# avik-pal/RegNeuralDE.jl

Hardware: AMD Instinct MI355X
Metric: training-step samples/sec + mean NFE, MNIST Neural ODE bs=512 (higher is better)
Workload: dtype f32; 1 GPU; MNIST NODE regularized (error_est), Tsit5 reltol=abstol=1.4e-8, batch 512 per GPU, 1xMI355X per rank; step = loss fwd + reverse pass through the solver + InvDecay/Momentum update; the weights train during the timed steps (mean_nfe drifts with --steps: value_fixed_weights of --full is the stationary companion); global_batch=512, parallelism=single

## Files before the change

regneuralde.jl_amd/csrc/rnde_reverse.hip:

```cpp
#include "rnde_node.h"
#include "rnde_wgradx.h"

static rnde_status chain_bwd_run(rnde_node* h, const float* u_bar_dev, const float* saveval_bar_host, float* x_bar_dev,
                                 float* p_bar_dev, float* tspan_bar_host, hipStream_t s, bool sync = true, float* tspan_bar_dev = nullptr);
static rnde_status bwd_run(rnde_node* h, const float* u_bar_dev, const float* saveval_bar_host, float* x_bar_dev,
                           float* p_bar_dev, float* tspan_bar_host, hipStream_t s, bool sync = true, float* tspan_bar_dev = nullptr);


extern "C" rnde_status rnde_node_backward_async(rnde_node* h, const float* u_bar_dev, const float* saveval_bar_host, float* x_bar_dev,
                                                float* p_bar_dev, float* tspan_bar_dev, void* stream) {
    if (!h) return RNDE_ERR_BAD_ARG;
    if (!h->have_tape) { h->err = "no recorded forward"; return RNDE_ERR_NO_TAPE; }
    if (h->engine == 3) return chain_bwd_run(h, u_bar_dev, saveval_bar_host, x_bar_dev, p_bar_dev, nullptr, (hipStream_t)stream, false, tspan_bar_dev);
    return bwd_run(h, u_bar_dev, saveval_bar_host, x_bar_dev, p_bar_dev, nullptr, (hipStream_t)stream, false, tspan_bar_dev);
}

extern "C" rnde_status rnde_node_backward(rnde_node* h, const float* u_bar_dev, const float* saveval_bar_host,
                                          float* x_bar_dev, float* p_bar_dev, float* tspan_bar_host, void* stream) {
    if (!h) return RNDE_ERR_BAD_ARG;
    if (!h->have_tape) { h->err = "no recorded forward"; return RNDE_ERR_NO_TAPE; }
    if (h->engine == 3) return chain_bwd_run(h, u_bar_dev, saveval_bar_host, x_bar_dev, p_bar_dev, tspan_bar_host, (hipStream_t)stream);
    return bwd_run(h, u_bar_dev, saveval_bar_host, x_bar_dev, p_bar_dev, tspan_bar_host, (hipStream_t)stream);
}
extern "C" rnde_status rnde_node_backward_host(rnde_node* h, const float* u_bar, const float* saveval_bar, float* x_bar,
                                               float* p_bar, float* tspan_bar) {
    if (!h) return RNDE_ERR_BAD_ARG;
    float *ub = nullptr, *xb = nullptr, *pb = nullptr;
    const size_t nb = (size_t)h->D * h->B * 4;
    HIPCHK(h, hipMalloc((void**)&ub, nb)); HIPCHK(h, hipMalloc((void**)&xb, nb)); HIPCHK(h, hipMalloc((void**)&pb, (size_t)h->P * 4));
    HIPCHK(h, hipMemcpy(ub, u_bar, nb, hipMemcpyHostToDevice));
    rnde_status st = rnde_node_backward(h, ub, saveval_bar, xb, pb, tspan_bar, nullptr);
    if (st == RNDE_OK) { hipMemcpy(x_bar, xb, nb, hipMemcpyDeviceToHost); hipMemcpy(p_bar, pb, (size_t)h->P * 4, hipMemcpyDeviceToHost); }
    hipFree(ub); hipFree(xb); hipFree(pb);
    return st;
}

static rnde_status bwd_prepare(rnde_node* h) {
    BwdBuffers& b = h->bw;
    if (b.ready) return RNDE_OK;
    const size_t A = (size_t)h->D * h->Bpad_max, HB = (size_t)h->H * h->Bpad_max;
    const int cap = h->cfg.max_attempts;
    HIPCHK(h, hipMalloc((void**)&b.U, A * 4)); HIPCHK(h, hipMalloc((void**)&b.K1, A * 4)); HIPCHK(h, hipMalloc((void**)&b.UB1, A * 4));
    HIPCHK(h, hipMalloc((void**)&b.zi2, 2 * A * 4)); HIPCHK(h, hipMalloc((void**)&b.zi1, 2 * HB * 4));
    HIPCHK(h, hipMalloc((void**)&b.svb_att, (size_t)cap * 4));
    HIPCHK(h, hipMalloc((void**)&b.bstate, 2 * sizeof(BState) + 64)); HIPCHK(h, hipMalloc((void**)&b.ibstate, 2 * sizeof(IBState)));
    HIPCHK(h, hipMalloc((void**)&b.bpart, (size_t)(2 * h->nwg_max + 256) * 4 * 4)); HIPCHK(h, hipMalloc((void**)&b.ipart, (size_t)2 * h->nwg_max * 4 * 4));
    HIPCHK(h, hipMalloc((void**)&b.tspan_out, 2 * 4));
    const size_t nev = (size_t)6 * cap + 2;
    const size_t desc_blob = 2 * nev * sizeof(EvalDesc) + (size_t)cap * 4 + 64;
    HIPCHK(h, hipMalloc((void**)&b.ev1, desc_blob)); HIPCHK(h, hipMalloc((void**)&b.ev2, nev * sizeof(EvalDesc)));
    HIPCHK(h, hipHostMalloc((void**)&b.h_ev1, desc_blob)); HIPCHK(h, hipHostMalloc((void**)&b.h_ev2, nev * sizeof(EvalDesc)));
    HIPCHK(h, hipHostMalloc((void**)&b.h_svb, (size_t)cap * 4));
    const size_t seg = std::max((size_t)h->H * (h->D + 2), (size_t)h->D * (h->H + 2));
    b.slab_floats = seg * 256;
    HIPCHK(h, hipMalloc((void**)&b.slab, 2 * b.slab_floats * 4));
    HIPCHK(h, hipMalloc((void**)&b.slab_r, 2 * 16 * seg * 4));
    if (!h->wstream) {
        int prio_least = 0, prio_greatest = 0;
        (void)hipDeviceGetStreamPriorityRange(&prio_least, &prio_greatest);
        HIPCHK(h, hipStreamCreateWithPriority(&h->wstream, hipStreamNonBlocking, prio_least));
        h->wevents.resize(66);
        for (auto& e : h->wevents) HIPCHK(h, hipEventCreateWithFlags(&e, hipEventDisableTiming));
    }
    if (h->engine == 2) {
        HIPCHK(h, hipMalloc((void**)&b.UTB, A * 4)); HIPCHK(h, hipMalloc((void**)&b.UNB, A * 4)); HIPCHK(h, hipMalloc((void**)&b.UPB0, A * 4));
        HIPCHK(h, hipMalloc((void**)&b.GB, 15 * A * 4));
    }
    b.ready = true;
    return RNDE_OK;
}

static bool wgrad3_ok(int M, int Nx) {
    const bool tall = M >= Nx;
    const int wide = tall ? M : Nx + 2, narrow = tall ? Nx + 2 : M;
    return getenv("RNDE_WGRAD_LEGACY") == nullptr && getenv("RNDE_WGRAD_V2") == nullptr && M % 4 == 0 && Nx % 4 == 0 && wide > 656 &&
           wide <= 800 && narrow <= 112;
}
static rnde_status launch_wgrad_part(rnde_node* h, const EvalDesc* ev, int n_evals, int per_chunk, int M, int Nx, int Bpad,
                                     float* slab, int* chunk_cursor, hipStream_t s, int max_chunks = 0) {
    if (n_evals <= 0) return RNDE_OK;
    const int mtiles = (M + 31) / 32, ntiles = (Nx + 2 + 31) / 32;
    const bool tall = M >= Nx;
    const int MB = tall ? 2 : 4, NB = tall ? 4 : 2;
    const int blocks = ((mtiles + MB - 1) / MB) * ((ntiles + NB - 1) / NB);
    const long long len = (long long)M * (Nx + 2);
    const int chunks = (n_evals + per_chunk - 1) / per_chunk;
    float* dst = slab + (size_t)(*chunk_cursor) * len;
    static const bool legacy = getenv("RNDE_WGRAD_LEGACY") != nullptr;
    const bool fits = tall ? (Nx + 2 <= 128) : (M <= 128);
    if (wgrad3_ok(M, Nx)) {
        const int total_steps = n_evals * ((Bpad + 31) / 32);
        static const int target_chunks = getenv("RNDE_WGRAD3_CHUNKS") ? atoi(getenv("RNDE_WGRAD3_CHUNKS")) : 128;
        int sc = std::max(1, std::min({max_chunks > 0 ? max_chunks : target_chunks, total_steps, 256}));
        const int steps_per_chunk = (total_steps + sc - 1) / sc;
        sc = (total_steps + steps_per_chunk - 1) / steps_per_chunk;
        if ((size_t)(*chunk_cursor + sc) * (size_t)len > h->bw.slab_floats) { h->err = "weight-gradient slab overflow"; return RNDE_ERR_BAD_ARG; }
        const bool x3_off = getenv("RNDE_X3_WGRAD_OFF") != nullptr;
        const bool x3_half = getenv("RNDE_X3_WGRAD_HALF") != nullptr;
        const int TT4 = ((tall ? M : Nx + 2) + 15) / 16;
        if (h->x3_packed && !x3_off && !x3_half && TT4 >= 28 && TT4 <= 52) {
            static const int target4 = getenv("RNDE_WGRAD4_CHUNKS") ? atoi(getenv("RNDE_WGRAD4_CHUNKS")) : 64;
            int sc4 = std::max(1, std::min({max_chunks > 0 ? max_chunks / 2 : target4, total_steps, 256}));
            const int spc4 = (total_steps + sc4 - 1) / sc4;
            sc4 = (total_steps + spc4 - 1) / spc4;
            if ((size_t)(*chunk_cursor + sc4) * (size_t)len > h->bw.slab_floats) { h->err = "weight-gradient slab overflow"; return RNDE_ERR_BAD_ARG; }
            static DeviceOnce attr4;
            if (attr4.need()) {
                HIPCHK(h, hipFuncSetAttribute((const void*)rnde_wgrad4x_kernel<true>, hipFuncAttributeMaxDynamicSharedMemorySize, (int)kWx4LdsBytes));
                HIPCHK(h, hipFuncSetAttribute((const void*)rnde_wgrad4x_kernel<false>, hipFuncAttributeMaxDynamicSharedMemorySize, (int)kWx4LdsBytes));
                attr4.done();
            }
            const dim3 g4(32 * ((sc4 + 7) / 8));
            if (tall) hipLaunchKernelGGL((rnde_wgrad4x_kernel<true>), g4, dim3(448), kWx4LdsBytes, s, ev, n_evals, spc4, sc4, M, Nx, Bpad, dst);
            else hipLaunchKernelGGL((rnde_wgrad4x_kernel<false>), g4, dim3(448), kWx4LdsBytes, s, ev, n_evals, spc4, sc4, M, Nx, Bpad, dst);
            HIPCHK(h, hipGetLastError());
            *chunk_cursor += sc4;
            return RNDE_OK;
        }
        if (h->x3_packed && !x3_off) {
            static DeviceOnce attrx;
            if (attrx.need()) {
                HIPCHK(h, hipFuncSetAttribute((const void*)rnde_wgrad3x_kernel<true>, hipFuncAttributeMaxDynamicSharedMemorySize, (int)kWxLdsBytes));
                HIPCHK(h, hipFuncSetAttribute((const void*)rnde_wgrad3x_kernel<false>, hipFuncAttributeMaxDynamicSharedMemorySize, (int)kWxLdsBytes));
                attrx.done();
            }
            if (tall) hipLaunchKernelGGL((rnde_wgrad3x_kernel<true>), dim3(2, sc), dim3(448), kWxLdsBytes, s, ev, n_evals, steps_per_chunk, M, Nx, Bpad, dst);
            else hipLaunchKernelGGL((rnde_wgrad3x_kernel<false>), dim3(2, sc), dim3(448), kWxLdsBytes, s, ev, n_evals, steps_per_chunk, M, Nx, Bpad, dst);
            HIPCHK(h, hipGetLastError());
            *chunk_cursor += sc;
            return RNDE_OK;
        }
        const size_t lds = (size_t)2 * 32 * (464 + 144) * sizeof(float);
        static DeviceOnce attr;
        if (attr.need()) {
            HIPCHK(h, hipFuncSetAttribute((const void*)rnde_wgrad3_kernel<true>, hipFuncAttributeMaxDynamicSharedMemorySize, (int)lds));
            HIPCHK(h, hipFuncSetAttribute((const void*)rnde_wgrad3_kernel<false>, hipFuncAttributeMaxDynamicSharedMemorySize, (int)lds));
            attr.done();
        }
        if (tall) hipLaunchKernelGGL((rnde_wgrad3_kernel<true>), dim3(2, sc), dim3(448), lds, s, ev, n_evals, steps_per_chunk, M, Nx, Bpad, dst);
        else hipLaunchKernelGGL((rnde_wgrad3_kernel<false>), dim3(2, sc), dim3(448), lds, s, ev, n_evals, steps_per_chunk, M, Nx, Bpad, dst);
        HIPCHK(h, hipGetLastError());
        *chunk_cursor += sc;
        return RNDE_OK;
    }
    if (!legacy && fits) {
        const int pblocks = tall ? (M + 127) / 128 : (Nx + 2 + 127) / 128;
        const int total_steps = n_evals * ((Bpad + 31) / 32);
        static const int target_wgs = getenv("RNDE_WGRAD_WGS") ? atoi(getenv("RNDE_WGRAD_WGS")) : 768;
        int sc = std::max(1, std::min({target_wgs / pblocks, total_steps, 256}));
        const int steps_per_chunk = (total_steps + sc - 1) / sc;
        sc = (total_steps + steps_per_chunk - 1) / steps_per_chunk;
        if ((size_t)(*chunk_cursor + sc) * (size_t)len > h->bw.slab_floats) { h->err = "weight-gradient slab overflow"; return RNDE_ERR_BAD_ARG; }
        if (tall) hipLaunchKernelGGL((rnde_wgrad2_kernel<true>), dim3(pblocks, sc), dim3(256), 0, s, ev, n_evals, steps_per_chunk, M, Nx, Bpad, dst);
        else hipLaunchKernelGGL((rnde_wgrad2_kernel<false>), dim3(pblocks, sc), dim3(256), 0, s, ev, n_evals, steps_per_chunk, M, Nx, Bpad, dst);
        HIPCHK(h, hipGetLastError());
        *chunk_cursor += sc;
        return RNDE_OK;
    } else {
        if ((size_t)(*chunk_cursor + chunks) * (size_t)len > h->bw.slab_floats) { h->err = "weight-gradient slab overflow"; return RNDE_ERR_BAD_ARG; }
        if (tall) hipLaunchKernelGGL((rnde_wgrad_kernel<2, 4>), dim3(blocks, chunks), dim3(64), 0, s, ev, n_evals, per_chunk, M, Nx, Bpad, dst);
        else hipLaunchKernelGGL((rnde_wgrad_kernel<4, 2>), dim3(blocks, chunks), dim3(64), 0, s, ev, n_evals, per_chunk, M, Nx, Bpad, dst);
    }
    HIPCHK(h, hipGetLastError());
    *chunk_cursor += chunks;
    return RNDE_OK;
}
static rnde_status launch_wgrad_reduce(rnde_node* h, const float* slab, int chunks, int M, int Nx, float* out, hipStream_t s) {
    const long long len = (long long)M * (Nx + 2);
    const int grid = (int)std::min<long long>((len + 255) / 256, 2048);
    if (chunks <= 16) {
        hipLaunchKernelGGL(rnde_wgrad_reduce, dim3(grid, 1), dim3(256), 0, s, slab, chunks, chunks, len, out);
    } else {
        const int per_group = (chunks + 15) / 16, groups = (chunks + per_group - 1) / per_group;
        hipLaunchKernelGGL(rnde_wgrad_reduce, dim3(grid, groups), dim3(256), 0, s, slab, chunks, per_group, len, h->bw.slab_r);
        hipLaunchKernelGGL(rnde_wgrad_reduce, dim3(grid, 1), dim3(256), 0, s, (const float*)h->bw.slab_r, groups, groups, len, out);
    }
    HIPCHK(h, hipGetLastError());
    return RNDE_OK;
}

static rnde_status bwd_run(rnde_node* h, const float* u_bar_dev, const float* saveval_bar_host, float* x_bar_dev,
                           float* p_bar_dev, float* tspan_bar_host, hipStream_t s, bool sync, float* tspan_bar_dev) {
    HIPCHK(h, hipSetDevice(h->cfg.device));
    rnde_status st = bwd_prepare(h);
    if (st != RNDE_OK) return st;
    BwdBuffers& b = h->bw;
    int n_att = h->n_att;
    const float svb_scale = h->couple ? (float)h->couple_world : 1.f;
    for (int i = 0; i < n_att; ++i)
        b.h_svb[i] = (saveval_bar_host && h->sv_index[i] >= 0) ? svb_scale * saveval_bar_host[h->sv_index[i]] : 0.f;
    const int ne_all = 2 + 6 * n_att;
    EvalDesc* const h_ev1 = b.h_ev1; EvalDesc* const h_ev2 = b.h_ev1 + ne_all; float* const h_svb_blob = (float*)(b.h_ev1 + 2 * (size_t)ne_all);
    EvalDesc* const d_ev1 = b.ev1;   EvalDesc* const d_ev2 = b.ev1 + ne_all;   float* const d_svb = (float*)(b.ev1 + 2 * (size_t)ne_all);
    memcpy(h_svb_blob, b.h_svb, (size_t)n_att * 4);
    BwdParams Q{};
    Q.F = make_params(h, h->xcopy, h->B, h->t0, h->t1, 1);
    Q.U = b.U; Q.K1 = b.K1; Q.UB1 = b.UB1; Q.zi2 = b.zi2; Q.zi1 = b.zi1; Q.svb_att = d_svb;
    Q.bstate = b.bstate; Q.ibstate = b.ibstate; Q.bpart = b.bpart; Q.ipart = b.ipart;
    Q.ubar = u_bar_dev; Q.xbar = x_bar_dev; Q.tspan_out = b.tspan_out;
    Q.n_att = n_att; Q.track_ctrl = h->cfg.track_ctrl; Q.track_initdt = h->cfg.track_initdt; Q.reg_kind = h->cfg.regularize;
    Q.bpart_n = Q.F.nwg;
    Q.tspan_scale = h->couple ? 1.f / (float)h->couple_world : 1.f;
#ifdef RNDE_DIAG
    if (getenv("RNDE_DIAG_BWD")) { if (!h->diag_buf) hipMalloc((void**)&h->diag_buf, 8192); hipMemset(h->diag_buf, 0, 512); Q.F.dbg_out = h->diag_buf; }
#endif
    Q.sv_T = (int)h->saveat.size();
    Q.sv_ubar0 = (!h->saveat.empty() && h->saveat[0] == h->t0) ? u_bar_dev : nullptr;
    if (!h->saveat.empty() && h->engine != 2) { h->err = "saveat reverse pass runs on the stage engine only"; return RNDE_ERR_BAD_ARG; }
    const long long A = (long long)h->D * Q.F.Bpad, HB = (long long)h->H * Q.F.Bpad;
    RecLayout L{A, HB};
    int ne = 2;
    h_ev2[0] = EvalDesc{b.zi2, h->h0, h->t0, 0};           h_ev1[0] = EvalDesc{b.zi1, h->xcopy, h->t0, 0};
    h_ev2[1] = EvalDesc{b.zi2 + A, h->h1, h->t0 + h->h_init->dt0, 0}; h_ev1[1] = EvalDesc{b.zi1 + HB, h->u1, h->t0 + h->h_init->dt0, 0};
    for (int n = 0; n < n_att; ++n) {
        const StepMeta& m = h->h_meta[n];
        const float* R = h->arena + (long long)m.rec * h->rec_stride;
        for (int sidx = 2; sidx <= 7; ++sidx) {
            const float ts = m.t + tsC(sidx - 1) * m.dt;
            h_ev2[ne] = EvalDesc{R + L.k(sidx), R + L.h(sidx), ts, 0};
            h_ev1[ne] = EvalDesc{R + L.z1(sidx), sidx < 7 ? R + L.g(sidx) : R + L.unew(), ts, 0};
            ++ne;
        }
    }
    HIPCHK(h, hipMemcpyAsync(b.ev1, b.h_ev1, 2 * (size_t)ne * sizeof(EvalDesc) + (size_t)n_att * 4, hipMemcpyHostToDevice, s));
    float* slab1 = b.slab;
    float* slab2w = b.slab + b.slab_floats;
    int cur1 = 0, cur2 = 0, evi = 0;
    const int per_chunk = std::max(1, (ne + 239) / 240);
    const int side_pct = h->wgrad_side_pct;
    const int sweep_cus = 8 * h->sR * ((Q.F.Bpad / 16 + 7) / 8);
    const bool side = h->engine == 2 && h->persist == 1 && side_pct > 0 && n_att >= 8 && sweep_cus <= 224 &&
                      wgrad3_ok(h->H, h->D) && wgrad3_ok(h->D, h->H);
    const int side_att = side ? std::min(n_att, n_att * side_pct / 100) : 0;
    const int group = std::max(4, (side_att + 5) / 6);
    bool used_side = false;
    auto wgrad_group = [&](int lo, int hi, bool on_side) -> rnde_status {
        if (hi <= lo) return RNDE_OK;
        hipStream_t ws = s;
        if (on_side) {
            hipEvent_t ev = h->wevents[evi++ % 64];
            HIPCHK(h, hipEventRecord(ev, s));
            HIPCHK(h, hipStreamWaitEvent(h->wstream, ev, 0));
            ws = h->wstream; used_side = true;
        }
        rnde_status r = launch_wgrad_part(h, d_ev1 + lo, hi - lo, per_chunk, h->H, h->D, h->B, slab1, &cur1, ws, on_side ? 16 : 0);
        if (r != RNDE_OK) return r;
        return launch_wgrad_part(h, d_ev2 + lo, hi - lo, per_chunk, h->D, h->H, h->B, slab2w, &cur2, ws, on_side ? 16 : 0);
    };
    int hi_att = n_att;
    hipError_t e;
    h->tev_bwd = false;
    if (h->timing) HIPCHK(h, hipEventRecord(h->tev[2], s));
    if (h->engine == 2) {
        if (!h->rev_packed) {
            HIPCHK(h, stage_pack(h, h->pcopy, h->spwBt, 2, h->sMT, h->sKHb, s));
            HIPCHK(h, stage_pack(h, h->pcopy, h->spwDt, 3, h->sHT, h->sMT, s));
        }
        h->rev_packed = false;
        BStageParams BQ{};
        BQ.B = Q; BQ.p = h->pcopy; BQ.pwBt = h->spwBt; BQ.pwDt = h->spwDt; BQ.slab = h->slab2; BQ.x3Bt = h->x3Bt; BQ.x3Dt = h->x3Dt;
        BQ.UTB = b.UTB; BQ.UNB = b.UNB; BQ.UPB0 = b.UPB0; BQ.GB = b.GB;
        BQ.EXK = b.GB + 6 * A; BQ.EXG = b.GB + 7 * A; BQ.SVW = b.GB + 8 * A;
        BQ.sv_t = h->saveat.empty() ? nullptr : h->sv_t_dev; BQ.sv_ubar = u_bar_dev; BQ.nsave = (int)h->saveat.size();
        BQ.MT = h->sMT; BQ.WT = h->sWT; BQ.R = h->sR; BQ.C = Q.F.Bpad / 16; BQ.HT = h->sHT; BQ.KHb = h->sKHb;
        double* const bsum = (double*)(b.bstate + 2);
        const bool pre_reduce = h->persist == 1 && Q.bpart_n >= 896 && !getenv("RNDE_NO_BPART_REDUCE");
        if (pre_reduce) BQ.B.bsum = bsum;
        const dim3 grid(BQ.R * BQ.C), blk(64 * BQ.WT);
        std::vector<int> sv_lo(n_att, 0), sv_hi(n_att, 0);
        if (!h->saveat.empty()) {
            int ns = (h->saveat[0] == h->t0) ? 1 : 0;
            for (int n = 0; n < n_att; ++n) {
                sv_lo[n] = ns;
                if (h->h_meta[n].flags & F_ACCEPT) {
                    const float tnew = h->h_meta[n].t + h->h_meta[n].dt;
                    while (ns < (int)h->saveat.size() && h->saveat[ns] <= tnew) ++ns;
                }
                sv_hi[n] = ns;
            }
        }
        auto eig_coefs = [&](int n, float& c1, float& c2) {
            c1 = 0.f; c2 = 0.f;
            const StepMeta& mm = h->h_meta[n];
            const bool eg_ok = !(mm.eigen == 0.f || mm.eigen != mm.eigen);
            double eigb = 0.0;
            if (h->cfg.regularize == RNDE_REG_STIFF && eg_ok) eigb = (double)b.h_svb[n] * (mm.eigen > 0 ? 1.0 : -1.0) / 3.5068;
            if (h->cfg.regularize == RNDE_REG_ERR_STIFF && eg_ok) eigb = 0.1 * (double)b.h_svb[n] / 3.5068;
            if (h->cfg.regularize == RNDE_REG_STIFF_DT && eg_ok) eigb = (double)b.h_svb[n] * ((double)mm.eigen * (double)mm.dt > 0 ? 1.0 : -1.0) * (double)mm.dt;
            if (eigb != 0.0 && mm.n1 > 0.f && mm.n2 > 0.f) {
                c1 = (float)(eigb / ((double)mm.n2 * (double)mm.n1));
                c2 = (float)(-eigb * ((double)mm.n1 / (double)mm.n2) / ((double)mm.n2 * (double)mm.n2));
            }
        };
        for (int n = n_att - 1; n >= 0; --n) {
            float c1 = 0.f, c2 = 0.f;
            eig_coefs(n, c1, c2);
            const double qo = pow((double)h->h_meta[n].qold_in, (double)kBeta2);
            if (h->persist == 1) {
                PersistSync Y{h->tslab, h->pabort, h->pxcc, h->persist_spins};
                HIPCHK(h, slab_prepare(h, Q.F.Bpad, s));
                const dim3 pgrid(8 * BQ.R * ((BQ.C + 7) / 8));
                const bool fix = BQ.WT == 7 && BQ.HT == 7 && BQ.KHb == 7 && BQ.MT == 49 && BQ.R == 7 && h->D == 784 && h->H == 100 && !h->stage_generic;
                if (fix) {
                    const size_t flds = h->stage_lds + (size_t)(RNDE_BSTAGE_HDMA ? 1 : 0) * 6 * 7 * 2 * 1024;
                    static DeviceOnce attr;
                    if (attr.need()) {
                        HIPCHK(h, hipFuncSetAttribute((const void*)rnde_bstage_attempt_kernel<1, 1>, hipFuncAttributeMaxDynamicSharedMemorySize, 160 * 1024));
                        HIPCHK(h, hipFuncSetAttribute((const void*)rnde_bstage_attempt_kernel<0, 1>, hipFuncAttributeMaxDynamicSharedMemorySize, 160 * 1024));
                        attr.done();
                    }
                    const bool x3 = h->x3_packed && h->x3Bt && h->x3Dt && !getenv("RNDE_X3_REV_OFF");
                    if (x3) {
                        const size_t xlds = sizeof(float) * ((size_t)2 * kX3ImageFloats + 64) + (size_t)(RNDE_BSTAGE_HDMA ? 1 : 0) * 6 * 7 * 2 * 1024;
                        static DeviceOnce attr3;
                        if (attr3.need()) {
#define RNDE_X3_ATTR(A, E) HIPCHK(h, hipFuncSetAttribute((const void*)rnde_bstage_attempt_kernel<A, 1, 1, E>, hipFuncAttributeMaxDynamicSharedMemorySize, 160 * 1024));
                            RNDE_X3_ATTR(1, 0) RNDE_X3_ATTR(1, 1) RNDE_X3_ATTR(1, 2) RNDE_X3_ATTR(1, 3) RNDE_X3_ATTR(0, 0) RNDE_X3_ATTR(0, 1) RNDE_X3_ATTR(0, 2) RNDE_X3_ATTR(0, 3)
#undef RNDE_X3_ATTR
                            attr3.done();
                        }
                        const int ex = (h->saveat.empty() ? 0 : 1) | (h->cfg.regularize >= RNDE_REG_STIFF ? 2 : 0);
#define RNDE_X3_LAUNCH(A, E) hipLaunchKernelGGL((rnde_bstage_attempt_kernel<A, 1, 1, E>), pgrid, blk, xlds, s, BQ, n, h->h_meta[n], c1, c2, sv_lo[n], sv_hi[n], Y, qo, b.h_svb[n])
                        if (h->act2) { if (ex == 0) RNDE_X3_LAUNCH(1, 0); else if (ex == 1) RNDE_X3_LAUNCH(1, 1); else if (ex == 2) RNDE_X3_LAUNCH(1, 2); else RNDE_X3_LAUNCH(1, 3); }
                        else { if (ex == 0) RNDE_X3_LAUNCH(0, 0); else if (ex == 1) RNDE_X3_LAUNCH(0, 1); else if (ex == 2) RNDE_X3_LAUNCH(0, 2); else RNDE_X3_LAUNCH(0, 3); }
#undef RNDE_X3_LAUNCH
                    } else if (h->act2) hipLaunchKernelGGL((rnde_bstage_attempt_kernel<1, 1>), pgrid, blk, flds, s, BQ, n, h->h_meta[n], c1, c2, sv_lo[n], sv_hi[n], Y, qo, b.h_svb[n]);
                    else hipLaunchKernelGGL((rnde_bstage_attempt_kernel<0, 1>), pgrid, blk, flds, s, BQ, n, h->h_meta[n], c1, c2, sv_lo[n], sv_hi[n], Y, qo, b.h_svb[n]);
                } else if (h->act2) hipLaunchKernelGGL((rnde_bstage_attempt_kernel<1, 0>), pgrid, blk, h->stage_lds, s, BQ, n, h->h_meta[n], c1, c2, sv_lo[n], sv_hi[n], Y, qo, b.h_svb[n]);
                else hipLaunchKernelGGL((rnde_bstage_attempt_kernel<0, 0>), pgrid, blk, h->stage_lds, s, BQ, n, h->h_meta[n], c1, c2, sv_lo[n], sv_hi[n], Y, qo, b.h_svb[n]);
                if ((st = couple_sum(h, b.bpart + (size_t)(n & 1) * Q.bpart_n * 4, 4LL * Q.bpart_n, s)) != RNDE_OK) return st;
                if (pre_reduce && n > 0) hipLaunchKernelGGL(rnde_bpart_reduce_kernel, dim3(1), dim3(64), 0, s, Q, n, bsum);
                if (n >= n_att - side_att && (hi_att - n >= group || n == n_att - side_att)) {
                    st = wgrad_group(2 + 6 * n, 2 + 6 * hi_att, true);
                    if (st != RNDE_OK) return st;
                    hi_att = n;
                }
                continue;
            }
            if (h->act2) hipLaunchKernelGGL((rnde_bstage_kernel<1, BM_START>), grid, blk, h->stage_lds, s, BQ, n, 0, h->h_meta[n], c1, c2, sv_lo[n], sv_hi[n], qo);
            else hipLaunchKernelGGL((rnde_bstage_kernel<0, BM_START>), grid, blk, h->stage_lds, s, BQ, n, 0, h->h_meta[n], c1, c2, sv_lo[n], sv_hi[n], qo);
            for (int j = 6; j >= 1; --j) {
                if (h->act2) hipLaunchKernelGGL((rnde_bstage_kernel<1, BM_STAGE>), grid, blk, h->stage_lds, s, BQ, n, j, h->h_meta[n], c1, c2, sv_lo[n], sv_hi[n], qo);
                else hipLaunchKernelGGL((rnde_bstage_kernel<0, BM_STAGE>), grid, blk, h->stage_lds, s, BQ, n, j, h->h_meta[n], c1, c2, sv_lo[n], sv_hi[n], qo);
            }
            if ((st = couple_sum(h, b.bpart + (size_t)(n & 1) * Q.bpart_n * 4, 4LL * Q.bpart_n, s)) != RNDE_OK) return st;
        }
        HIPCHK(h, hipGetLastError());
        {
            if (h->act2) {
                hipLaunchKernelGGL((rnde_binit_stage_kernel<1, 0>), grid, blk, h->stage_lds, s, BQ);
                hipLaunchKernelGGL((rnde_binit_stage_kernel<1, 1>), grid, blk, h->stage_lds, s, BQ);
            } else {
                hipLaunchKernelGGL((rnde_binit_stage_kernel<0, 0>), grid, blk, h->stage_lds, s, BQ);
                hipLaunchKernelGGL((rnde_binit_stage_kernel<0, 1>), grid, blk, h->stage_lds, s, BQ);
            }
            if ((st = couple_sum(h, Q.ipart, 4LL * Q.F.nwg, s)) != RNDE_OK) return st;
            if (h->act2) {
                hipLaunchKernelGGL((rnde_binit_stage_kernel<1, 2>), grid, blk, h->stage_lds, s, BQ);
                hipLaunchKernelGGL((rnde_binit_stage_kernel<1, 3>), grid, blk, h->stage_lds, s, BQ);
            } else {
                hipLaunchKernelGGL((rnde_binit_stage_kernel<0, 2>), grid, blk, h->stage_lds, s, BQ);
                hipLaunchKernelGGL((rnde_binit_stage_kernel<0, 3>), grid, blk, h->stage_lds, s, BQ);
            }
            if ((st = couple_sum(h, Q.ipart + 4LL * Q.F.nwg, 4LL * Q.F.nwg, s)) != RNDE_OK) return st;
            hipLaunchKernelGGL(rnde_bfin_kernel, dim3(1), dim3(64), 0, s, Q);
            HIPCHK(h, hipGetLastError());
        }
    }
    if (h->timing) HIPCHK(h, hipEventRecord(h->tev[3], s));
    st = wgrad_group(0, 2 + 6 * hi_att, false);
    if (st != RNDE_OK) return st;
    if (used_side) {
        hipEvent_t ev = h->wevents[64];
        HIPCHK(h, hipEventRecord(ev, h->wstream));
        HIPCHK(h, hipStreamWaitEvent(s, ev, 0));
    }
    if (cur1 > 16 && cur2 > 16) {
        const long long len1 = (long long)h->H * (h->D + 2), len2 = (long long)h->D * (h->H + 2);
        const size_t seg_r = std::max((size_t)len1, (size_t)len2);
        float* r1 = b.slab_r; float* r2 = b.slab_r + 16 * seg_r;
        const int pg1 = (cur1 + 15) / 16, g1 = (cur1 + pg1 - 1) / pg1, pg2 = (cur2 + 15) / 16, g2 = (cur2 + pg2 - 1) / pg2;
        const int grid = (int)std::min<long long>((std::max(len1, len2) + 255) / 256, 2048);
        ReducePair A{{{slab1, r1, len1, cur1, pg1}, {slab2w, r2, len2, cur2, pg2}}};
        hipLaunchKernelGGL(rnde_wgrad_reduce_pair, dim3(grid, std::max(g1, g2), 2), dim3(256), 0, s, A);
        ReducePair Bp{{{r1, p_bar_dev, len1, g1, g1}, {r2, p_bar_dev + (size_t)h->H * (h->D + 2), len2, g2, g2}}};
        hipLaunchKernelGGL(rnde_wgrad_reduce_pair, dim3(grid, 1, 2), dim3(256), 0, s, Bp);
        HIPCHK(h, hipGetLastError());
    } else {
        st = launch_wgrad_reduce(h, slab1, cur1, h->H, h->D, p_bar_dev, s);
        if (st != RNDE_OK) return st;
        st = launch_wgrad_reduce(h, slab2w, cur2, h->D, h->H, p_bar_dev + (size_t)h->H * (h->D + 2), s);
        if (st != RNDE_OK) return st;
    }
    if (h->timing) { HIPCHK(h, hipEventRecord(h->tev[4], s)); h->tev_bwd = true; }
#ifdef RNDE_DIAG
    if (h->engine == 2 && h->persist == 1 && getenv("RNDE_DIAG_BWD")) {
        unsigned long long hst[64] = {0};
        hipStreamSynchronize(s);
        hipMemcpy(hst, h->diag_buf, sizeof(hst), hipMemcpyDeviceToHost);
        fprintf(stderr, "persistent reverse attempt (workgroup 0 thread 0, cycles): START %lld (entry->weights issued %lld, ->w1t %lld, ->array loads issued %lld, finish_attempt_scalars %lld, scalar chain %lld, vector part %lld), its phase D + put %lld\n", (long long)(hst[1]-hst[0]), (long long)(hst[43]-hst[0]), (long long)(hst[44]-hst[43]), (long long)(hst[40]-hst[44]), (long long)(hst[41]-hst[40]), (long long)(hst[42]-hst[41]), (long long)(hst[1]-hst[42]), (long long)(hst[2]-hst[1]));
        for (int st = 0; st < 6; ++st) { const unsigned long long* q = hst + 3 + 5 * st; const unsigned long long prev = st == 0 ? hst[2] : hst[7 + 5 * (st - 1)];
            fprintf(stderr, "  stage j=%d: poll %lld A %lld B %lld C %lld D+put %lld\n", 6 - st, (long long)(q[0]-prev), (long long)(q[1]-q[0]), (long long)(q[2]-q[1]), (long long)(q[3]-q[2]), st < 5 ? (long long)(q[4]-q[3]) : 0LL); }
        fprintf(stderr, "  total %lld cycles to the end of stage 1, END (reduction of the 21 partial sums) %lld; in START's vector part the wait for the record's k arrays %lld\n",
                (long long)(hst[34]-hst[0]), (long long)(hst[35]-hst[34]), (long long)(hst[45]-hst[42]));
    }
#endif
    if (!sync) {
        if (tspan_bar_dev) HIPCHK(h, hipMemcpyAsync(tspan_bar_dev, b.tspan_out, 8, hipMemcpyDeviceToDevice, s));
        h->have_tape = false;
        h->pending_bwd = (h->engine == 2 && h->persist == 1);
        return RNDE_OK;
    }
    HIPCHK(h, hipMemcpyAsync(h->h_scal, b.tspan_out, 8, hipMemcpyDeviceToHost, s));
    if (h->engine == 2) persist_check_enqueue(h, h->sR * (Q.F.Bpad / 16), s);
    HIPCHK(h, hipStreamSynchronize(s));
    if (h->couple && rnde_comm_health(h->couple) != RNDE_OK) { h->err = std::string("coupled controller: ") + rnde_comm_last_error(h->couple); return RNDE_ERR_HIP; }
    if (tspan_bar_host) { tspan_bar_host[0] = h->h_scal[0]; tspan_bar_host[1] = h->h_scal[1]; }
// ... 406 lines not shown
```

regneuralde.jl_amd/csrc/rnde_wgradx.h:

```cpp
#pragma once
#include "rnde_x3.h"

namespace rnde {

constexpr int kWxRowShorts = 40;
constexpr int kWxTallRows = 400, kWxNarrowRows = 112;
constexpr int kWxPlaneShortsT = kWxTallRows * kWxRowShorts, kWxPlaneShortsS = kWxNarrowRows * kWxRowShorts;
constexpr size_t kWxLdsBytes = (size_t)3 * (kWxPlaneShortsT + kWxPlaneShortsS) * 2;

template <bool TALL_IS_Z>
__global__ __launch_bounds__(448) void rnde_wgrad3x_kernel(const EvalDesc* __restrict__ evals, int n_evals, int per_chunk, int M, int Nx, int Bpad, float* __restrict__ slab) {
    constexpr int KC = 32;
    extern __shared__ __attribute__((aligned(16))) unsigned short wxs[];
    unsigned short* TP = wxs;
    unsigned short* SP = wxs + 3 * kWxPlaneShortsT;
    const int tid = threadIdx.x, lane = tid & 63, w = __builtin_amdgcn_readfirstlane(tid >> 6);
    const int mrow = lane & 15, kk = lane >> 4;
    const int TR = TALL_IS_Z ? M : Nx + 2, SR = TALL_IS_Z ? Nx + 2 : M;
    const int TRp = TALL_IS_Z ? M : Nx, SRp = TALL_IS_Z ? Nx : M;
    const int TT = (TR + 15) >> 4, T0 = (TT + 1) >> 1;
    const int half = blockIdx.x, chunk = blockIdx.y;
    const int tile_lo = half ? T0 : 0, tile_hi = half ? TT : T0, ntile = tile_hi - tile_lo;
    const int row_lo = 16 * tile_lo, nrow = 16 * ntile;
    const int steps_per_eval = (Bpad + KC - 1) / KC;
    const int s_lo = chunk * per_chunk, s_hi = min(n_evals * steps_per_eval, s_lo + per_chunk);
    const int total_steps = max(0, s_hi - s_lo);
    x3f4 acc[4][7];
#pragma unroll
    for (int i = 0; i < 4; ++i)
#pragma unroll
        for (int n = 0; n < 7; ++n) acc[i][n] = (x3f4){0.f, 0.f, 0.f, 0.f};
    const bool has3 = w + 21 < ntile;

    constexpr unsigned kNoSrc = 0x7FFFFF00u;
    int u_kind[5], u_dst[5];
    unsigned u_voff[5];
#pragma unroll
    for (int jj = 0; jj < 4; ++jj) {
        const int u = tid + 448 * jj;
        int kind = 0, dst = 0; unsigned voff = kNoSrc;
        if (u < 4 * nrow) {
            const int o = u / nrow, row = u - o * nrow, gr = row_lo + row;
            kind = gr < TRp ? 1 : (!TALL_IS_Z && gr == TRp ? 2 : (!TALL_IS_Z && gr == TRp + 1 ? 3 : 4));
            if (kind == 1) voff = 4u * (unsigned)(gr + 8 * o * TRp);
            dst = row * kWxRowShorts + 8 * o;
        }
        u_kind[jj] = kind; u_voff[jj] = voff; u_dst[jj] = dst;
    }
    {
        const int o = tid / kWxNarrowRows, row = tid - o * kWxNarrowRows;
        const int kind = row < SRp ? 1 : (TALL_IS_Z && row == SRp ? 2 : (TALL_IS_Z && row == SRp + 1 ? 3 : 4));
        u_kind[4] = kind; u_voff[4] = kind == 1 ? 4u * (unsigned)(row + 8 * o * SRp) : kNoSrc;
        u_dst[4] = 3 * kWxPlaneShortsT + row * kWxRowShorts + 8 * o;
    }
    int e_nx = s_lo / steps_per_eval, cs_nx = s_lo - e_nx * steps_per_eval;
    float stg[5][8];
    float stg_t = 0.f; int stg_ncols = 0;
    auto fetch = [&]() {
        const int e = e_nx, c0 = cs_nx * KC;
        if (++cs_nx == steps_per_eval) { cs_nx = 0; ++e_nx; }
        stg_t = evals[e].t;
        stg_ncols = min(KC, Bpad - c0);
        __amdgpu_buffer_rsrc_t rsT = __builtin_amdgcn_make_buffer_rsrc((void*)(TALL_IS_Z ? evals[e].Z : evals[e].X), 0, 4 * TRp * Bpad, 0x00020000);
        __amdgpu_buffer_rsrc_t rsS = __builtin_amdgcn_make_buffer_rsrc((void*)(TALL_IS_Z ? evals[e].X : evals[e].Z), 0, 4 * SRp * Bpad, 0x00020000);
#pragma unroll
        for (int jj = 0; jj < 5; ++jj) {
            const int cs = jj < 4 ? TRp : SRp;
#pragma unroll
            for (int j = 0; j < 8; ++j) {
                const unsigned off = u_voff[jj] + 4u * (unsigned)((c0 + j) * cs);
                stg[jj][j] = __builtin_bit_cast(float, __builtin_amdgcn_raw_buffer_load_b32(jj < 4 ? rsT : rsS, (int)off, 0, 2));
            }
        }
    };
    auto spill = [&]() {
#pragma unroll
        for (int jj = 0; jj < 5; ++jj) {
            const int kind = u_kind[jj];
            if (kind == 0) continue;
            const int o8 = u_dst[jj] % kWxRowShorts;
            float v[8];
#pragma unroll
            for (int j = 0; j < 8; ++j) v[j] = kind == 1 ? stg[jj][j] : ((kind == 2 || kind == 3) && o8 + j < stg_ncols ? (kind == 2 ? stg_t : 1.f) : 0.f);
            unsigned hi[4], mid[4], lo[4];
#pragma unroll
            for (int j = 0; j < 4; ++j) x3_split2(v[2 * j], v[2 * j + 1], hi[j], mid[j], lo[j]);
            unsigned short* d = wxs + u_dst[jj];
            const int ps = jj < 4 ? kWxPlaneShortsT : kWxPlaneShortsS;
            *(x3u4*)d = (x3u4){hi[0], hi[1], hi[2], hi[3]};
            *(x3u4*)(d + ps) = (x3u4){mid[0], mid[1], mid[2], mid[3]};
            *(x3u4*)(d + 2 * ps) = (x3u4){lo[0], lo[1], lo[2], lo[3]};
        }
    };
    auto fragT = [&](int tile, int pl) { return *(const x3u4*)(TP + pl * kWxPlaneShortsT + (16 * tile + mrow) * kWxRowShorts + 8 * kk); };
    auto fragS = [&](int tile, int pl) { return *(const x3u4*)(SP + pl * kWxPlaneShortsS + (16 * tile + mrow) * kWxRowShorts + 8 * kk); };

    if (total_steps > 0) { fetch(); spill(); }
    __syncthreads();
    for (int step = 0; step < total_steps; ++step) {
        if (step + 1 < total_steps) fetch();
#pragma unroll
        for (int ps = 0; ps < 2; ++ps) {
            x3u4 a[2][3];
#pragma unroll
            for (int i = 0; i < 2; ++i) {
                const int ii = 2 * ps + i, tile = (ii < 3 || has3) ? w + 7 * ii : w;
#pragma unroll
                for (int pl = 0; pl < 3; ++pl) a[i][pl] = fragT(tile, pl);
            }
#pragma unroll
            for (int n = 0; n < 7; ++n) {
                __builtin_amdgcn_sched_barrier(0);
                const x3u4 bh = fragS(n, 0), bm = fragS(n, 1), bl = fragS(n, 2);
#define WX_TERM(PA, BV) _Pragma("unroll") for (int i = 0; i < 2; ++i) if (2 * ps + i < 3 || has3) acc[2 * ps + i][n] = x3_mfma(a[i][PA], BV, acc[2 * ps + i][n]);
                WX_TERM(2, bh) WX_TERM(0, bl) WX_TERM(1, bm) WX_TERM(1, bh) WX_TERM(0, bm) WX_TERM(0, bh)
#undef WX_TERM
            }
        }
        __syncthreads();
        if (step + 1 < total_steps) spill();
        __syncthreads();
    }
    float* out = slab + (size_t)chunk * M * (Nx + 2);
#pragma unroll
    for (int i = 0; i < 4; ++i) {
        if (w + 7 * i < ntile) {
#pragma unroll
            for (int n = 0; n < 7; ++n) {
                const int sr = 16 * n + mrow;
#pragma unroll
                for (int q = 0; q < 4; ++q) {
                    const int tr = row_lo + 16 * (w + 7 * i) + 4 * kk + q;
                    if (tr < TR && sr < SR) out[TALL_IS_Z ? (size_t)sr * M + tr : (size_t)tr * M + sr] = acc[i][n][q];
                }
            }
        }
    }
}

#ifndef RNDE_WX4_SB
#define RNDE_WX4_SB 1
#endif
#ifndef RNDE_WX4_ABL
#define RNDE_WX4_ABL 0
#endif
constexpr int kWx4TallRows = 208;
constexpr int kWx4PlaneT = kWx4TallRows * kWxRowShorts, kWx4PlaneS = kWxNarrowRows * kWxRowShorts;
constexpr int kWx4ImageShorts = 3 * (kWx4PlaneT + kWx4PlaneS);
constexpr size_t kWx4LdsBytes = (size_t)2 * kWx4ImageShorts * 2;

template <bool TALL_IS_Z>
__global__ __launch_bounds__(448) void rnde_wgrad4x_kernel(const EvalDesc* __restrict__ evals, int n_evals, int per_chunk, int n_chunks, int M, int Nx, int Bpad,
                                                           float* __restrict__ slab) {
    constexpr int KC = 32;
    extern __shared__ __attribute__((aligned(16))) unsigned short wxs[];
    const int tid = threadIdx.x, lane = tid & 63, w = __builtin_amdgcn_readfirstlane(tid >> 6);
    const int mrow = lane & 15, kk = lane >> 4;
    const int lin = blockIdx.x, xcd = lin & 7, within = lin >> 3;
    const int chunk = (within >> 2) * 8 + xcd, part = within & 3;
    if (chunk >= n_chunks) return;
    const int TR = TALL_IS_Z ? M : Nx + 2, SR = TALL_IS_Z ? Nx + 2 : M;
    const int TRp = TALL_IS_Z ? M : Nx, SRp = TALL_IS_Z ? Nx : M;
    const int TT = (TR + 15) >> 4, base = TT >> 2, rem = TT & 3;
    const int ntile = base + (part < rem ? 1 : 0), tile_lo = part * base + (part < rem ? part : rem);
    const int row_lo = 16 * tile_lo, nrow = 16 * ntile;
    const int steps_per_eval = (Bpad + KC - 1) / KC;
    const int s_lo = chunk * per_chunk, s_hi = min(n_evals * steps_per_eval, s_lo + per_chunk);
    const int total_steps = max(0, s_hi - s_lo);
    x3f4 acc[2][7];
#pragma unroll
    for (int i = 0; i < 2; ++i)
#pragma unroll
        for (int n = 0; n < 7; ++n) acc[i][n] = (x3f4){0.f, 0.f, 0.f, 0.f};
    const bool has2 = w + 7 < ntile;
    const int tile1 = has2 ? w + 7 : w;

    constexpr unsigned kNoSrc = 0x7FFFFF00u;
    const bool wide_wave = w < 4;
    const int Rp = wide_wave ? TRp : SRp;
    const int nunit = wide_wave ? nrow : kWxNarrowRows;
    const int uid = (wide_wave ? tid : tid - 256) % nunit;
    const int uq = uid >> 2, uo = uid & 3;
    const int u_gr = (wide_wave ? row_lo : 0) + 4 * uq;
    const bool u_mem = u_gr < Rp;
    const bool u_syn = u_gr == Rp && (wide_wave ? !TALL_IS_Z : TALL_IS_Z);
    const float syn_f = u_syn ? 1.f : 0.f;
    const unsigned u_voff = u_mem ? 4u * (unsigned)(u_gr + 8 * uo * Rp) : kNoSrc;
    const int u_dst = (wide_wave ? 0 : 3 * kWx4PlaneT) + 4 * uq * kWxRowShorts + 8 * uo;
    const int u_ps = wide_wave ? kWx4PlaneT : kWx4PlaneS;
    int e_nx = s_lo / steps_per_eval, cs_nx = s_lo - e_nx * steps_per_eval, left = total_steps;
    x3f4 stg[2][8];
    float stg_t[2] = {0.f, 0.f}; int stg_ncols[2] = {0, 0};
    auto fetch = [&](auto set_c) {
        constexpr int SET = decltype(set_c)::value;
        const int e = e_nx, c0 = cs_nx * KC;
        {
            const bool adv = --left > 0, wrap = cs_nx + 1 == steps_per_eval;
            e_nx = (adv && wrap) ? e_nx + 1 : e_nx;
            cs_nx = adv ? (wrap ? 0 : cs_nx + 1) : cs_nx;
        }
        stg_t[SET] = evals[e].t;
        stg_ncols[SET] = min(KC, Bpad - c0);
        const float* src = wide_wave == TALL_IS_Z ? evals[e].Z : evals[e].X;
        __amdgpu_buffer_rsrc_t rs = __builtin_amdgcn_make_buffer_rsrc((void*)src, 0, 4 * Rp * Bpad, 0x00020000);
#pragma unroll
        for (int j = 0; j < 8; ++j)
            stg[SET][j] = __builtin_bit_cast(x3f4, __builtin_amdgcn_raw_buffer_load_b128(rs, (int)u_voff, 4 * (c0 + j) * Rp, 0));
    };
    unsigned abl_sink = 0u;
    auto spill_row = [&](unsigned short* img, int i, auto set_c) {
        constexpr int SET = decltype(set_c)::value;
        float v[8];
#pragma unroll
        for (int j = 0; j < 8; ++j) v[j] = i < 2 ? stg[SET][j][i] + (i == 0 ? syn_f * stg_t[SET] : syn_f) : stg[SET][j][i];
        unsigned hi[4], mid[4], lo[4];
#if RNDE_WX4_ABL == 6
#pragma unroll
        for (int j = 0; j < 4; ++j) { hi[j] = __float_as_uint(v[2 * j]); mid[j] = __float_as_uint(v[2 * j + 1]); lo[j] = hi[j]; }
#else
#pragma unroll
        for (int j = 0; j < 4; ++j) x3_split2(v[2 * j], v[2 * j + 1], hi[j], mid[j], lo[j]);
#endif
        unsigned short* d = img + u_dst + i * kWxRowShorts;
#if RNDE_WX4_ABL == 5
        abl_sink ^= hi[0] ^ hi[1] ^ hi[2] ^ hi[3] ^ mid[0] ^ mid[1] ^ mid[2] ^ mid[3] ^ lo[0] ^ lo[1] ^ lo[2] ^ lo[3];
        (void)d;
#else
        *(x3u4*)d = (x3u4){hi[0], hi[1], hi[2], hi[3]};
        *(x3u4*)(d + u_ps) = (x3u4){mid[0], mid[1], mid[2], mid[3]};
        *(x3u4*)(d + 2 * u_ps) = (x3u4){lo[0], lo[1], lo[2], lo[3]};
#endif
    };
    unsigned short* const img0 = wxs;
    unsigned short* const img1 = wxs + kWx4ImageShorts;
    if (total_steps == 0) return;
    typedef std::integral_constant<int, 0> S0;
    typedef std::integral_constant<int, 1> S1;
    fetch(S0{});
#pragma unroll
    for (int i = 0; i < 4; ++i) spill_row(img0, i, S0{});
    fetch(S0{});
    fetch(S1{});
    __syncthreads();
    auto one_step = [&](const unsigned short* cur, unsigned short* nxt, auto more_c, auto set_c) {
        constexpr bool MORE = decltype(more_c)::value;
        const unsigned short* SPc = cur + 3 * kWx4PlaneT;
        auto fragT = [&](int tile, int pl) { return *(const x3u4*)(cur + pl * kWx4PlaneT + (16 * tile + mrow) * kWxRowShorts + 8 * kk); };
        auto fragS = [&](int tile, int pl) { return *(const x3u4*)(SPc + pl * kWx4PlaneS + (16 * tile + mrow) * kWxRowShorts + 8 * kk); };
        x3u4 a[2][3];
#pragma unroll
        for (int pl = 0; pl < 3; ++pl) { a[0][pl] = fragT(w, pl); a[1][pl] = fragT(tile1, pl); }
        x3u4 bh = fragS(0, 0), bm = fragS(0, 1), bl = fragS(0, 2);
#pragma unroll
        for (int n = 0; n < 7; ++n) {
            x3u4 nh = bh, nm = bm, nl = bl;
#if RNDE_WX4_ABL != 3 && RNDE_WX4_ABL != 4
            if (n < 6) { nh = fragS(n + 1, 0); nm = fragS(n + 1, 1); nl = fragS(n + 1, 2); }
#endif
#if RNDE_WX4_ABL != 1 && RNDE_WX4_ABL != 2 && RNDE_WX4_ABL != 4
            if (MORE && n < 4) spill_row(nxt, n, set_c);
#endif
#if RNDE_WX4_ABL != 2 && RNDE_WX4_ABL != 4
            if (MORE && n == 4) fetch(set_c);
#endif
#define WX4_TERM(PA, BV) { acc[0][n] = x3_mfma(a[0][PA], BV, acc[0][n]); acc[1][n] = x3_mfma(a[1][PA], BV, acc[1][n]); }
            WX4_TERM(2, bh) WX4_TERM(0, bl) WX4_TERM(1, bm) WX4_TERM(1, bh) WX4_TERM(0, bm) WX4_TERM(0, bh)
#undef WX4_TERM
            bh = nh; bm = nm; bl = nl;
#if RNDE_WX4_SB
            __builtin_amdgcn_sched_barrier(0);
#endif
        }
    };
    int step = 0;
    for (; step + 2 < total_steps; step += 2) {
        one_step(img0, img1, std::true_type{}, S0{});
        __syncthreads();
        one_step(img1, img0, std::true_type{}, S1{});
        __syncthreads();
    }
    if (total_steps - step == 2) {
        one_step(img0, img1, std::true_type{}, S0{});
        __syncthreads();
        one_step(img1, nullptr, std::false_type{}, S1{});
    } else one_step(img0, nullptr, std::false_type{}, S0{});
#if RNDE_WX4_ABL == 5
    if (abl_sink == 0x12345678u) slab[0] = 1.f;
#endif
    float* out = slab + (size_t)chunk * M * (Nx + 2);
#pragma unroll
    for (int i = 0; i < 2; ++i) {
        if (w + 7 * i < ntile) {
#pragma unroll
            for (int n = 0; n < 7; ++n) {
                const int sr = 16 * n + mrow;
#pragma unroll
                for (int q = 0; q < 4; ++q) {
                    const int tr = row_lo + 16 * (w + 7 * i) + 4 * kk + q;
                    if (tr < TR && sr < SR) out[TALL_IS_Z ? (size_t)sr * M + tr : (size_t)tr * M + sr] = acc[i][n][q];
                }
            }
        }
    }
}

}
```

Measured before the change: 306,300 samples/s.

## Add swizzled LDS feed layout for wgrad4x kernel and make it default

Adds a FEED template variant of the wgrad4x weight-gradient kernel that stores the three split-precision planes in a packed 32-short-row, XOR-swizzled LDS layout, with remapped thread-to-row assignment for the global loads and precomputed fragment offsets for the MFMA reads. The intent is to remove LDS bank conflicts and padding waste in the spill and fragment-read paths. Default feed is 1, so the new layout runs unless an env var selects the old one. It adds index complexity and the risk of a mis-swizzle producing wrong gradients.

```diff
diff --git a/regneuralde.jl_amd/csrc/rnde_reverse.hip b/regneuralde.jl_amd/csrc/rnde_reverse.hip
--- a/regneuralde.jl_amd/csrc/rnde_reverse.hip
+++ b/regneuralde.jl_amd/csrc/rnde_reverse.hip
@@ -106,13 +106,24 @@
             if ((size_t)(*chunk_cursor + sc4) * (size_t)len > h->bw.slab_floats) { h->err = "weight-gradient slab overflow"; return RNDE_ERR_BAD_ARG; }
             static DeviceOnce attr4;
             if (attr4.need()) {
-                HIPCHK(h, hipFuncSetAttribute((const void*)rnde_wgrad4x_kernel<true>, hipFuncAttributeMaxDynamicSharedMemorySize, (int)kWx4LdsBytes));
-                HIPCHK(h, hipFuncSetAttribute((const void*)rnde_wgrad4x_kernel<false>, hipFuncAttributeMaxDynamicSharedMemorySize, (int)kWx4LdsBytes));
+                HIPCHK(h, hipFuncSetAttribute((const void*)rnde_wgrad4x_kernel<true, 0>, hipFuncAttributeMaxDynamicSharedMemorySize, (int)kWx4LdsBytes));
+                HIPCHK(h, hipFuncSetAttribute((const void*)rnde_wgrad4x_kernel<false, 0>, hipFuncAttributeMaxDynamicSharedMemorySize, (int)kWx4LdsBytes));
+                HIPCHK(h, hipFuncSetAttribute((const void*)rnde_wgrad4x_kernel<true, 1>, hipFuncAttributeMaxDynamicSharedMemorySize, (int)kWx4fLdsBytes));
+                HIPCHK(h, hipFuncSetAttribute((const void*)rnde_wgrad4x_kernel<false, 1>, hipFuncAttributeMaxDynamicSharedMemorySize, (int)kWx4fLdsBytes));
                 attr4.done();
             }
             const dim3 g4(32 * ((sc4 + 7) / 8));
-            if (tall) hipLaunchKernelGGL((rnde_wgrad4x_kernel<true>), g4, dim3(448), kWx4LdsBytes, s, ev, n_evals, spc4, sc4, M, Nx, Bpad, dst);
-            else hipLaunchKernelGGL((rnde_wgrad4x_kernel<false>), g4, dim3(448), kWx4LdsBytes, s, ev, n_evals, spc4, sc4, M, Nx, Bpad, dst);
+#if RNDE_WX4_ABL == 7 || RNDE_WX4_ABL == 8
+            const bool q0 = true;
+#else
+            const char* ef = getenv("RNDE_X3_WGRAD_FEED");
+            const bool q0 = getenv("RNDE_X3_WGRAD_Q0") != nullptr || (ef ? ef[0] == '0' : kWx4DefaultFeed == 0);
+#endif
+            if (q0) {
+                if (tall) hipLaunchKernelGGL((rnde_wgrad4x_kernel<true, 0>), g4, dim3(448), kWx4LdsBytes, s, ev, n_evals, spc4, sc4, M, Nx, Bpad, dst);
+                else hipLaunchKernelGGL((rnde_wgrad4x_kernel<false, 0>), g4, dim3(448), kWx4LdsBytes, s, ev, n_evals, spc4, sc4, M, Nx, Bpad, dst);
+            } else if (tall) hipLaunchKernelGGL((rnde_wgrad4x_kernel<true, 1>), g4, dim3(448), kWx4fLdsBytes, s, ev, n_evals, spc4, sc4, M, Nx, Bpad, dst);
+            else hipLaunchKernelGGL((rnde_wgrad4x_kernel<false, 1>), g4, dim3(448), kWx4fLdsBytes, s, ev, n_evals, spc4, sc4, M, Nx, Bpad, dst);
             HIPCHK(h, hipGetLastError());
             *chunk_cursor += sc4;
             return RNDE_OK;
diff --git a/regneuralde.jl_amd/csrc/rnde_wgradx.h b/regneuralde.jl_amd/csrc/rnde_wgradx.h
--- a/regneuralde.jl_amd/csrc/rnde_wgradx.h
+++ b/regneuralde.jl_amd/csrc/rnde_wgradx.h
@@ -148,8 +148,14 @@
 constexpr int kWx4PlaneT = kWx4TallRows * kWxRowShorts, kWx4PlaneS = kWxNarrowRows * kWxRowShorts;
 constexpr int kWx4ImageShorts = 3 * (kWx4PlaneT + kWx4PlaneS);
 constexpr size_t kWx4LdsBytes = (size_t)2 * kWx4ImageShorts * 2;
-
-template <bool TALL_IS_Z>
+constexpr int kWx4fRowShorts = 32;
+constexpr int kWx4fWideShorts = (kWx4TallRows + 4) * kWx4fRowShorts;
+constexpr int kWx4fPlane = (kWx4TallRows + 4 + kWxNarrowRows + 4) * kWx4fRowShorts;
+constexpr int kWx4fImageShorts = 3 * kWx4fPlane;
+constexpr size_t kWx4fLdsBytes = (size_t)2 * kWx4fImageShorts * 2;
+constexpr int kWx4DefaultFeed = 1;
+
+template <bool TALL_IS_Z, int FEED>
 __global__ __launch_bounds__(448) void rnde_wgrad4x_kernel(const EvalDesc* __restrict__ evals, int n_evals, int per_chunk, int n_chunks, int M, int Nx, int Bpad,
                                                            float* __restrict__ slab) {
     constexpr int KC = 32;
@@ -179,15 +185,43 @@
     const bool wide_wave = w < 4;
     const int Rp = wide_wave ? TRp : SRp;
     const int nunit = wide_wave ? nrow : kWxNarrowRows;
-    const int uid = (wide_wave ? tid : tid - 256) % nunit;
-    const int uq = uid >> 2, uo = uid & 3;
-    const int u_gr = (wide_wave ? row_lo : 0) + 4 * uq;
-    const bool u_mem = u_gr < Rp;
+    const int ut = wide_wave ? tid : tid - 256;
+    const int nquad = nunit >> 2;
+    const bool u_real = ut < nunit;
+    const int uid = ut % nunit;
+    const int uq = FEED ? uid % nquad : uid >> 2, uo = FEED ? uid / nquad : uid & 3;
+#if RNDE_WX4_ABL == 7
+    const int lq = uid % nquad, lo8 = uid / nquad;
+#else
+    const int lq = uq, lo8 = uo;
+#endif
+    const int u_gr = (wide_wave ? row_lo : 0) + 4 * lq;
+#if RNDE_WX4_ABL == 8
+    const bool u_mem = u_gr < Rp && u_real;
+#else
+    const bool u_mem = u_gr < Rp && (FEED == 0 || u_real);
+#endif
     const bool u_syn = u_gr == Rp && (wide_wave ? !TALL_IS_Z : TALL_IS_Z);
     const float syn_f = u_syn ? 1.f : 0.f;
-    const unsigned u_voff = u_mem ? 4u * (unsigned)(u_gr + 8 * uo * Rp) : kNoSrc;
+    const unsigned u_voff = u_mem ? 4u * (unsigned)(u_gr + 8 * lo8 * Rp) : kNoSrc;
+#if RNDE_WX4_ABL == 8
+    const int u_dst = (wide_wave ? 0 : 3 * kWx4PlaneT) + 4 * uq * kWxRowShorts + (u_real ? 8 * uo : 32);
+#else
     const int u_dst = (wide_wave ? 0 : 3 * kWx4PlaneT) + 4 * uq * kWxRowShorts + 8 * uo;
+#endif
     const int u_ps = wide_wave ? kWx4PlaneT : kWx4PlaneS;
+    int f_dst[4] = {0, 0, 0, 0};
+    int f_frag[2] = {0, 0};
+    if (FEED) {
+        const int qa = u_real ? uq & 3 : lane & 3, qt = u_real ? (uq >> 2) & 1 : (lane >> 2) & 1, qo = u_real ? uo : 0;
+        const int line = (wide_wave ? 0 : kWx4fWideShorts) + 128 * (u_real ? uq : wide_wave ? kWx4TallRows / 4 : kWxNarrowRows / 4);
+#pragma unroll
+        for (int b = 0; b < 4; ++b) f_dst[b] = line + 32 * ((b + qa) & 3) + 8 * ((qo ^ (4 - qa) ^ qt) & 3);
+        const int fa = mrow >> 2;
+        f_frag[0] = 128 * fa + 32 * ((mrow + fa) & 3) + 8 * ((kk ^ (4 - fa)) & 3);
+        f_frag[1] = f_frag[0] ^ 8;
+    }
+    const int f_a0 = f_frag[w & 1] + 512 * w, f_a1 = f_frag[tile1 & 1] + 512 * tile1;
     int e_nx = s_lo / steps_per_eval, cs_nx = s_lo - e_nx * steps_per_eval, left = total_steps;
     x3f4 stg[2][8];
     float stg_t[2] = {0.f, 0.f}; int stg_ncols[2] = {0, 0};
@@ -221,18 +255,19 @@
 #pragma unroll
         for (int j = 0; j < 4; ++j) x3_split2(v[2 * j], v[2 * j + 1], hi[j], mid[j], lo[j]);
 #endif
-        unsigned short* d = img + u_dst + i * kWxRowShorts;
+        unsigned short* d = FEED ? img + f_dst[i] : img + u_dst + i * kWxRowShorts;
+        const int ps = FEED ? kWx4fPlane : u_ps;
 #if RNDE_WX4_ABL == 5
         abl_sink ^= hi[0] ^ hi[1] ^ hi[2] ^ hi[3] ^ mid[0] ^ mid[1] ^ mid[2] ^ mid[3] ^ lo[0] ^ lo[1] ^ lo[2] ^ lo[3];
         (void)d;
 #else
         *(x3u4*)d = (x3u4){hi[0], hi[1], hi[2], hi[3]};
-        *(x3u4*)(d + u_ps) = (x3u4){mid[0], mid[1], mid[2], mid[3]};
-        *(x3u4*)(d + 2 * u_ps) = (x3u4){lo[0], lo[1], lo[2], lo[3]};
+        *(x3u4*)(d + ps) = (x3u4){mid[0], mid[1], mid[2], mid[3]};
+        *(x3u4*)(d + 2 * ps) = (x3u4){lo[0], lo[1], lo[2], lo[3]};
 #endif
     };
     unsigned short* const img0 = wxs;
-    unsigned short* const img1 = wxs + kWx4ImageShorts;
+    unsigned short* const img1 = wxs + (FEED ? kWx4fImageShorts : kWx4ImageShorts);
     if (total_steps == 0) return;
     typedef std::integral_constant<int, 0> S0;
     typedef std::integral_constant<int, 1> S1;
@@ -244,12 +279,18 @@
     __syncthreads();
     auto one_step = [&](const unsigned short* cur, unsigned short* nxt, auto more_c, auto set_c) {
         constexpr bool MORE = decltype(more_c)::value;
-        const unsigned short* SPc = cur + 3 * kWx4PlaneT;
-        auto fragT = [&](int tile, int pl) { return *(const x3u4*)(cur + pl * kWx4PlaneT + (16 * tile + mrow) * kWxRowShorts + 8 * kk); };
-        auto fragS = [&](int tile, int pl) { return *(const x3u4*)(SPc + pl * kWx4PlaneS + (16 * tile + mrow) * kWxRowShorts + 8 * kk); };
+        const unsigned short* SPc = cur + (FEED ? kWx4fWideShorts : 3 * kWx4PlaneT);
+        auto fragT = [&](int i, int pl) {
+            if (FEED) return *(const x3u4*)(cur + pl * kWx4fPlane + (i ? f_a1 : f_a0));
+            return *(const x3u4*)(cur + pl * kWx4PlaneT + (16 * (i ? tile1 : w) + mrow) * kWxRowShorts + 8 * kk);
+        };
+        auto fragS = [&](int tile, int pl) {
+            if (FEED) return *(const x3u4*)(SPc + pl * kWx4fPlane + f_frag[tile & 1] + 512 * tile);
+            return *(const x3u4*)(SPc + pl * kWx4PlaneS + (16 * tile + mrow) * kWxRowShorts + 8 * kk);
+        };
         x3u4 a[2][3];
 #pragma unroll
-        for (int pl = 0; pl < 3; ++pl) { a[0][pl] = fragT(w, pl); a[1][pl] = fragT(tile1, pl); }
+        for (int pl = 0; pl < 3; ++pl) { a[0][pl] = fragT(0, pl); a[1][pl] = fragT(1, pl); }
         x3u4 bh = fragS(0, 0), bm = fragS(0, 1), bl = fragS(0, 2);
 #pragma unroll
         for (int n = 0; n < 7; ++n) {
```

Result: faster. 310,900 samples/s, median of 6 (+1.5%).
